# yhlleo/DWC-GAN

Hardware: AMD Instinct MI355X
Metric: CelebA 128x128 training images/sec (higher is better)
Workload: dtype f32; 1 GPU; BASELINE configs[1]: CelebA-shaped 128x128, per-GPU batch 16, fp32, full iteration (dis_update + gen_update + EMA + LR step), vgg_w=0, stride-1 3x3 / 5x5 and stride-2 4x4 layers (forward, data and weight gradient) as fp32-accurate TWO-plane f16 split products on the f16 MFMA (hi + lo 2^-11 per operand, per-tensor power-of-two scales, 3 products per multiply-add, matrix-core partial sums flushed to; image_size=128, per_gpu_batch=16, global_batch=16, parallelism=dp1

## Files before the change

### dwc-gan_amd/hipdwc/_lib.py

```python
import ctypes
import os

_HERE = os.path.dirname(os.path.abspath(__file__))
LIB_PATH = os.environ.get("DWC_HIP_LIB") or os.path.join(os.path.dirname(_HERE), "lib", "libdwcgan_hip.so")

c_fp = ctypes.c_void_p
c_int = ctypes.c_int
c_sz = ctypes.c_size_t
c_f = ctypes.c_float
c_u = ctypes.c_uint


class AdvSpec(ctypes.Structure):
    _fields_ = [("target", c_f * 4), ("w_src", c_f * 4), ("w_cls", c_f * 4)]


BN_MAX_SEGMENTS = 8


class BnOrder(ctypes.Structure):
    _fields_ = [("n", c_int), ("idx", c_int * BN_MAX_SEGMENTS)]


SIGNATURES = {
    "dwc_version": (c_int, []),
    "dwc_x3_gemm_mode": (c_int, [c_int]),
    "dwc_weight_prepared_elems": (c_sz, [c_int] * 8),
    "dwc_weight_prepare_fwd": (c_int, [c_fp, c_fp, c_int, c_int, c_int, c_int, c_int, c_int, c_fp]),
    "dwc_weight_prepare_dgrad": (c_int, [c_fp, c_fp, c_int, c_int, c_int, c_int, c_int, c_int, c_int, c_fp]),
    "dwc_conv2d_fwd_ws_bytes": (c_sz, [c_int] * 9),
    "dwc_conv2d_fwd": (c_int, [c_fp, c_fp, c_fp, c_fp] + [c_int] * 10 + [c_fp, c_sz, c_fp]),
    "dwc_conv2d_bwd_data_ws_bytes": (c_sz, [c_int] * 9),
# ... 183 lines not shown
    "dwc_bf16_conv2d_bwd_weight_plan": (c_int, [c_int] * 9 + [c_fp]),
    "dwc_conv2d_bwd_weight_zeropad_ws_bytes": (c_sz, [c_int] * 9),
    "dwc_conv2d_bwd_weight_zeropad": (c_int, [c_fp, c_fp, c_fp] + [c_int] * 11 + [c_fp, c_sz, c_fp]),
    "dwc_conv2d_bwd_data_crop_ws_bytes": (c_sz, [c_int] * 9),
    "dwc_conv2d_bwd_data_crop": (c_int, [c_fp, c_fp, c_fp] + [c_int] * 9 + [c_fp, c_sz, c_fp]),
    "dwc_bf16_conv2d_bwd_weight_zeropad_ws_bytes": (c_sz, [c_int] * 9),
    "dwc_bf16_conv2d_bwd_weight_zeropad": (c_int, [c_fp, c_fp, c_fp] + [c_int] * 11 + [c_fp, c_sz, c_fp]),
    "dwc_bf16_conv2d_bwd_data_crop_ws_bytes": (c_sz, [c_int] * 9),
    "dwc_bf16_conv2d_bwd_data_crop": (c_int, [c_fp, c_fp, c_fp] + [c_int] * 9 + [c_fp, c_sz, c_fp]),
    "dwc_x3_conv2d_wgrad_zeropad": (c_int, [c_fp, c_fp, c_fp] + [c_int] * 8 + [c_fp, c_sz, c_fp]),
    "dwc_h2_conv2d_wgrad_zeropad": (c_int, [c_fp, c_fp, c_u, c_fp, c_fp, c_u, c_fp] + [c_int] * 8 + [c_fp, c_sz, c_fp]),
    "dwc_bf16_conv2d_wgrad_halo_zeropad": (c_int, [c_fp, c_fp, c_fp] + [c_int] * 8 + [c_fp, c_sz, c_fp]),
    "dwc_x3_conv2d_s2_ws_zeropad": (c_int, [c_fp] * 4 + [c_int] * 7 + [c_fp, c_sz, c_fp, c_fp]),
    "dwc_h2_conv2d_s2_ws_zeropad": (c_int, [c_fp, c_fp, c_u, c_fp, c_fp, c_fp, c_fp, c_u] + [c_int] * 7 + [c_fp, c_sz, c_fp, c_fp]),
    "dwc_bf16_conv2d_s2_halo_zeropad": (c_int, [c_fp, c_fp, c_fp, c_fp] + [c_int] * 6 + [c_fp]),
}

ABI_VERSION = 11
EINVAL = -1
_ERRORS = {-1: "DWC_EINVAL (unsupported shape/argument)", -2: "DWC_EWORKSPACE (scratch too small)",
           -3: "DWC_ELAUNCH (kernel launch failed)"}

_lib = None


class HipKernelError(RuntimeError):
    pass


def load():
# ... 35 lines not shown
```

### dwc-gan_amd/hipdwc/ops.py

```python
import os
import weakref

import numpy as np
import torch

from . import _lib

ACT = {"none": 0, None: 0, "relu": 1, "lrelu": 2, "tanh": 3, "sigmoid": 4, "heads": 5, "heads8": 6}

PRECISION = "fp32"
BF16 = torch.bfloat16

_REMOVED_SWITCHES = ("DWC_WINOGRAD", "DWC_TXT_STREAM", "DWC_NORM_FUSED_FINAL", "DWC_GEMM_TILE", "DWC_STRIP_BM", "DWC_X3_DUO", "DWC_X3_BN",
                     "DWC_X3_BN32", "DWC_X3_WIDE", "DWC_X3_STAGGER", "DWC_HALO_STAGGER", "DWC_X3_WDUO", "DWC_HALO16", "DWC_HALO_DUO",
                     "DWC_HALO_BN128", "DWC_BF16_TILE", "DWC_BF16_STAGES3", "DWC_NARROW_ROWS16")
_set = [k for k in _REMOVED_SWITCHES if k in os.environ]
if _set:
    import warnings
    warnings.warn("hipdwc: %s no longer select%s anything (removed in round 5, DESIGN.md 10.3) and %s ignored" % (
        ", ".join(_set), "s" if len(_set) == 1 else "", "is" if len(_set) == 1 else "are"), stacklevel=2)
del _set


def set_precision(name):
# ... 1433 lines not shown
    K = w.shape[1]
    c = _pow2_div(N)
    taps = N // c
    wt4 = w.detach().t().reshape(K, taps, c).permute(0, 2, 1).unsqueeze(3)
    wp = _prepped(wt4, "fwd", K, c, 1, owner)
    dx = torch.empty((M, K), dtype=torch.float32, device=dy.device)
    nws = lib.dwc_conv2d_fwd_ws_bytes(M, taps, 1, c, K, taps, 1, 1, 0)
    wsp = workspace(nws, dy.device).data_ptr() if nws else None
    flops = 2.0 * M * N * K
    _lib.check(_timed("conv_gemm_kernel", flops, lambda: lib.dwc_conv2d_fwd(
        dy.data_ptr(), wp.data_ptr(), None, dx.data_ptr(), M, taps, 1, c, K, taps, 1, 1, 0, 0, wsp, nws, _stream()),
        detail="dgrad B%d %dx1 %d>%d k%d s1" % (M, taps, c, K, taps)), "gemm_nn")
    return dx


def _gemm_tn(dy, x, out=None):
    lib = _lib.load()
    M, N = dy.shape
    K = x.shape[1]
    c = _pow2_div(K)
    taps = K // c
    dw4 = torch.empty((N, c, 1, taps), dtype=torch.float32, device=x.device)
    nws = lib.dwc_conv2d_bwd_weight_ws_bytes(M, 1, taps, c, N, 1, taps, 1, 0)
    ws = workspace(nws, x.device)
    flops = 2.0 * M * N * K
    _lib.check(_timed("conv_wgrad_kernel+reduce", flops, lambda: lib.dwc_conv2d_bwd_weight(
        x.data_ptr(), dy.data_ptr(), dw4.data_ptr(), M, 1, taps, c, N, 1, taps, 1, 0, c, N, ws.data_ptr(), ws.numel(), _stream()),
        detail="wgrad B%d 1x%d %d>%d k%d s1" % (M, taps, c, N, taps)), "gemm_tn")
    if out is None:
        return dw4.squeeze(2).permute(0, 2, 1).reshape(N, K)
    out.view(N, taps, c).copy_(dw4.squeeze(2).permute(0, 2, 1))
    return out


class _LinearAny(torch.autograd.Function):

    @staticmethod
    def forward(ctx, x, w, b, owner):
        _require_device(x)
        if x.dtype != torch.float32 or not gemm_ok(x.shape[1], w.shape[0]):
            raise ValueError("linear_any: fp32, widths multiples of 4 (got %s x %s)" % (tuple(x.shape), tuple(w.shape)))
        x = x.contiguous()
        ctx.owner = owner if owner is not None else w
# ... 3 lines not shown

    @staticmethod
    def backward(ctx, dy):
        x, w = ctx.saved_tensors
        dy = dy.contiguous()
        dx = _gemm_nn(dy, w, ctx.owner) if ctx.needs_input_grad[0] else None
        dw = _gemm_tn(dy, x) if ctx.needs_input_grad[1] else None
        db = dy.sum(0) if (ctx.has_b and ctx.needs_input_grad[2]) else None
        return dx, dw, db, None


def linear_any(x, w, b, owner=None):
    return _LinearAny.apply(x, w, b, owner)


LSTM_GEMM = int(os.environ.get("DWC_LSTM_GEMM", "1"))
_LSTM_STATUS = {}
LSTM_SEQ_MAX_WORKGROUPS = 0


def _lstm_status(device):
    key = device.index if device.index is not None else torch.cuda.current_device()
    ent = _LSTM_STATUS.get(key)
    if ent is None:
        ent = [torch.zeros(1, dtype=torch.int32, device=device), torch.zeros(1, dtype=torch.int32).pin_memory(), None]
        _LSTM_STATUS[key] = ent
    return ent


def lstm_status_poll(device, wait=False):
# ... 2 lines not shown
    ent = _lstm_status(device)
    if ent[2] is not None and (wait or ent[2].query()):
        if wait:
            ent[2].synchronize()
        if int(ent[1][0]) != 0:
            raise _lib.HipKernelError(
                "persistent LSTM kernel: a workgroup hand-off timed out (status %d: not all workgroups of the launch were resident); "
                "its results were overwritten with NaN.  Re-run with DWC_LSTM_SEQ=0 (per-step kernels)." % int(ent[1][0]))
        ent[2] = None
    if ent[2] is None:
        ent[1].copy_(ent[0], non_blocking=True)
        ent[2] = torch.cuda.Event()
        ent[2].record()


class _LSTMBidir(torch.autograd.Function):

    @staticmethod
    def forward(ctx, x, lens, w_ih, w_hh, b_ih, b_hh, owners=None):
        _require_device(x)
        lib = _lib.load()
        T, B, I = x.shape
        H = w_hh.shape[2]
        dev = x.device
        X = x.reshape(T * B, I)
        ctx.hip_gemm = bool(LSTM_GEMM and owners is not None and gemm_ok(I, 4 * H) and gemm_ok(H, 4 * H))
        ctx.owners = owners
        if ctx.hip_gemm:
            bsum = b_ih + b_hh
            X = X.contiguous()
            xproj = torch.empty((2, T * B, 4 * H), dtype=torch.float32, device=dev)
            for d in range(2):
                _gemm_nt(X, w_ih[d], bsum[d], owners[d], out=xproj[d])
        else:
            xproj = torch.baddbmm((b_ih + b_hh).unsqueeze(1), X.unsqueeze(0).expand(2, -1, -1), w_ih.transpose(1, 2))
        w_hh_c = w_hh.contiguous()
        out = torch.empty((2, T, B, H), dtype=torch.float32, device=dev)
        c = torch.empty((2, T, B, H), dtype=torch.float32, device=dev)
        gates = torch.empty((2, T, B, 4 * H), dtype=torch.float32, device=dev)
        rc = -1
        if LSTM_SEQ:
            ws = workspace(lib.dwc_lstm_seq_ws_bytes(B, 2), dev)
            rc = lib.dwc_lstm_seq_fwd(xproj.data_ptr(), w_hh_c.data_ptr(), lens.data_ptr(), out.data_ptr(), c.data_ptr(),
                                      gates.data_ptr(), T, B, H, 2, ws.data_ptr(), ws.numel(), _lstm_status(dev)[0].data_ptr(),
                                      LSTM_SEQ_MAX_WORKGROUPS, _stream())
            if rc not in (0, _lib.EINVAL):
                _lib.check(rc, "lstm_seq_fwd")
        if rc != 0:
            _lib.check(lib.dwc_lstm_fwd(xproj.data_ptr(), w_hh_c.data_ptr(), lens.data_ptr(), out.data_ptr(), c.data_ptr(),
                                        gates.data_ptr(), T, B, H, 2, _stream()), "lstm_fwd")
        ctx.save_for_backward(X, lens, w_ih, w_hh_c, out, c, gates)
        ctx.shape = (T, B, I, H)
        return out, c

    @staticmethod
    def backward(ctx, d_out, d_c):
        lib = _lib.load()
        X, lens, w_ih, w_hh, out, c, gates = ctx.saved_tensors
        T, B, I, H = ctx.shape
        dev = X.device
        d_out = None if d_out is None else d_out.contiguous()
        d_c = None if d_c is None else d_c.contiguous()
        w_hh_t = w_hh.transpose(1, 2).contiguous()
        dgates = torch.empty((2, T, B, 4 * H), dtype=torch.float32, device=dev)
        carry = torch.empty((2, B, H), dtype=torch.float32, device=dev)
        rc = -1
        if LSTM_SEQ:
            ws = workspace(lib.dwc_lstm_seq_ws_bytes(B, 2), dev)
            rc = lib.dwc_lstm_seq_bwd(_p(d_out), _p(d_c), w_hh_t.data_ptr(), lens.data_ptr(), c.data_ptr(), gates.data_ptr(),
                                      dgates.data_ptr(), T, B, H, 2, ws.data_ptr(), ws.numel(), _lstm_status(dev)[0].data_ptr(),
                                      LSTM_SEQ_MAX_WORKGROUPS, _stream())
            if rc not in (0, _lib.EINVAL):
                _lib.check(rc, "lstm_seq_bwd")
        if rc != 0:
            _lib.check(lib.dwc_lstm_bwd(_p(d_out), _p(d_c), w_hh_t.data_ptr(), lens.data_ptr(), c.data_ptr(), gates.data_ptr(),
                                        dgates.data_ptr(), carry.data_ptr(), T, B, H, 2, _stream()), "lstm_bwd")
        dG = dgates.view(2, T * B, 4 * H)
        dGt = dG.transpose(1, 2)
        hip = ctx.hip_gemm
        dw_ih = None
        if ctx.needs_input_grad[2]:
            if hip:
                dw_ih = torch.empty((2, 4 * H, I), dtype=torch.float32, device=dev)
                for d in range(2):
                    _gemm_tn(dG[d], X, out=dw_ih[d])
            else:
                dw_ih = torch.matmul(dGt, X)
        db = dG.sum(1) if (ctx.needs_input_grad[4] or ctx.needs_input_grad[5]) else None
        dw_hh = None
        if ctx.needs_input_grad[3]:
            hprev = torch.zeros((2, T, B, H), dtype=torch.float32, device=dev)
            hprev[0, 1:] = out[0, :-1]
            hprev[1, :-1] = out[1, 1:]
            hp = hprev.view(2, T * B, H)
            if hip:
                dw_hh = torch.empty((2, 4 * H, H), dtype=torch.float32, device=dev)
                for d in range(2):
                    _gemm_tn(dG[d], hp[d], out=dw_hh[d])
            else:
                dw_hh = torch.bmm(dGt, hp)
        dx = None
        if ctx.needs_input_grad[0]:
            if hip:
                dx = (_gemm_nn(dG[0], w_ih[0], ctx.owners[0]) + _gemm_nn(dG[1], w_ih[1], ctx.owners[1])).view(T, B, I)
            else:
                dx = torch.bmm(dG, w_ih).sum(0).view(T, B, I)
        return dx, None, dw_ih, dw_hh, db, db, None


def lstm_bidir(x, lens, w_ih, w_hh, b_ih, b_hh, owners=None):
    return _LSTMBidir.apply(x.contiguous(), lens, w_ih, w_hh, b_ih, b_hh, owners)


def _norm_call(name, x, out, args):
    lib = _lib.load()
    slot, ep = out_amax(out)
    if slot is None:
        _lib.check(_fn(lib, name, x)(*args, _stream()), name)
        return None
    _lib.check(getattr(lib, "dwc_%s_amax" % name)(*args, slot, ep, _stream()), name)
    return slot, ep


class _InstNorm(torch.autograd.Function):
    @staticmethod
    def forward(ctx, x, gamma, beta, residual, act, eps, token=None):
# ... 355 lines not shown
```

### dwc-gan_amd/networks/networks_v2.py

```python
import numpy as np
import torch
from torch import nn

from hipdwc import host, ops
from .networks import ContentEncoder, MLP, Conv2dBlock, ResBlocks, AdaptiveInstanceNorm2d, Decoder


class HeadList(list):
    flat = None

    @classmethod
    def of(cls, flat, k):
        out = cls(flat.reshape(flat.shape[0], k, -1).unbind(1))
        out.flat = flat
        return out

    def rows(self, a, b):
        return HeadList.of(self.flat[a:b], len(self))


def flat_heads(heads):
    if torch.is_tensor(heads):
        return heads
    flat = getattr(heads, "flat", None)
# ... 76 lines not shown
            table = np.zeros((vocab.size, embed_dim))
            for i, word in enumerate(vocab.itos):
                table[i] = pretrained_embed[word] if word in pretrained_embed else \
                    np.random.normal(scale=0.6, size=(embed_dim,))
            self.embed_tokens.load_state_dict({"weight": torch.from_numpy(table)})
            self.embed_tokens.weight.requires_grad = False
        self.lstm = nn.LSTM(input_size=embed_dim + self.style_dim, hidden_size=hidden_size, num_layers=num_layers,
                            dropout=dropout_out if num_layers > 1 else 0.0, bidirectional=bidirectional)
        feat = hidden_size * num_layers * (4 if bidirectional else 2)
        self.fcs, self.fcvars = nn.ModuleList(), nn.ModuleList()
        for _ in range(num_class):
            self.fcs.append(nn.Linear(feat, c_dim))
            self.fcvars.append(nn.Linear(feat, c_dim))

    def forward(self, style_ord, src_tokens, src_lengths):
        noise = host.noise()
        tokens = src_tokens.transpose(1, 0)
        seq_len, bsz = tokens.shape
        lens_host = src_lengths.detach().to("cpu")
        lens_sorted, order_host = torch.sort(lens_host, descending=True)
        if tokens.is_cuda and ops.PINNED_STAGE:
            stage = torch.empty(4, bsz, dtype=torch.int64).pin_memory()
            stage[0], stage[1], stage[2], stage[3] = order_host, torch.sort(order_host)[1], lens_sorted, lens_sorted - 1
            on_dev = stage.to(tokens.device, non_blocking=True)
            order, unsort, lens_dev, last = on_dev[0], on_dev[1], on_dev[2].to(torch.int32), on_dev[3]
        else:
            order, unsort = order_host.to(tokens.device), torch.sort(order_host)[1].to(tokens.device)
            lens_dev, last = lens_sorted.to(torch.int32).to(tokens.device), (lens_sorted - 1).to(tokens.device)
        emb = self.embed_tokens(tokens.index_select(1, order))
        emb = noise.dropout(emb, self.dropout_in, self.training)
        sty = _Permute.apply(style_ord, 0, order, unsort)
        lens_list = lens_sorted.tolist()
        t_max = int(lens_list[0])
        data = torch.cat([emb, sty.expand(seq_len, -1, -1)], -1)[:t_max]
        cols = torch.arange(bsz, device=tokens.device)
        suffixes = ("", "_reverse") if self.bidirectional else ("",)
        if not self.bidirectional:
            raise NotImplementedError("the HIP text encoder is bidirectional (the reference's only configuration)")
        hs, cs = [], []
        for l in range(self.num_layers):
            par = {n: ops.cat_params([getattr(self.lstm, "%s_l%d%s" % (n, l, suf)) for suf in suffixes], stack=True)
                   for n in ("weight_ih", "weight_hh", "bias_ih", "bias_hh")}
            out, cell = ops.lstm_bidir(data, lens_dev, par["weight_ih"], par["weight_hh"], par["bias_ih"], par["bias_hh"],
                                       owners=tuple(getattr(self.lstm, "weight_ih_l%d%s" % (l, suf)) for suf in suffixes))
            hs += [out[0][last, cols], out[1][0]]
            cs += [cell[0][last, cols], cell[1][0]]
            data = torch.cat([out[0], out[1]], -1)
            if l + 1 < self.num_layers and self.training and self.dropout_out > 0:
                if getattr(noise, "align_stream", False):
                    mask = noise.dropout_mask((int(sum(lens_list)), data.shape[2]), self.dropout_out, data.device)
                    data = data * mask.index_select(0, _packed_index(lens_list, t_max, bsz, data.device)).view(t_max, bsz, -1)
                else:
                    data = noise.dropout(data, self.dropout_out, True)
        h_n, c_n = torch.stack(hs), torch.stack(cs)
        if self.training and self.dropout_out > 0 and noise.align_stream:
            noise.dropout(data, self.dropout_out, True)
        h_n = h_n.view(self.num_layers, 2, bsz, -1).transpose(1, 2).reshape(self.num_layers, bsz, -1)
        c_n = c_n.view(self.num_layers, 2, bsz, -1).transpose(1, 2).reshape(self.num_layers, bsz, -1)
        h_n, c_n = _Permute.apply(h_n, 1, unsort, order), _Permute.apply(c_n, 1, unsort, order)
        feat = torch.cat([h_n, c_n], dim=1).view(bsz, -1)
        w = ops.cat_params([m.weight for m in self.fcs] + [m.weight for m in self.fcvars])
        b = ops.cat_params([m.bias for m in self.fcs] + [m.bias for m in self.fcvars])
        if feat.is_cuda and ops.LSTM_GEMM and ops.gemm_ok(feat.shape[1], w.shape[0]):
            out = ops.linear_any(feat, w, b, owner=tuple(m.weight for m in self.fcs) + tuple(m.weight for m in self.fcvars))
        else:
            out = torch.nn.functional.linear(feat, w, b)
        k, c = self.num_class, self.style_dim // self.num_class
        return HeadList.of(out[:, :k * c], k), HeadList.of(out[:, k * c:2 * k * c], k)


class AdaINGen_v2(nn.Module):

    def __init__(self, input_dim, vocab, params, pretrained_embed=None):
        super().__init__()
        p = params
# ... 58 lines not shown
```

### include/dwcgan_hip.h

```cpp
#ifndef DWCGAN_HIP_H
#define DWCGAN_HIP_H

#include <stddef.h>
#include <stdint.h>

#ifdef __cplusplus
extern "C" {
#endif

#define DWC_OK 0
#define DWC_EINVAL (-1)
#define DWC_EWORKSPACE (-2)
#define DWC_ELAUNCH (-3)

#define DWC_ACT_NONE 0
#define DWC_ACT_RELU 1
#define DWC_ACT_LRELU 2
#define DWC_ACT_TANH 3
#define DWC_ACT_SIGMOID 4
#define DWC_ACT_HEADS 5
#define DWC_ACT_HEADS8 6

#define DWC_ABI_VERSION 11
int dwc_version(void);
// ... 413 lines not shown
                      float* dx, float* dgamma, float* dbeta, int S, int Bs, int HW, int C, int act, int training, void* ws,
                      size_t ws_bytes, void* stream);
int dwc_batchnorm_fwd_amax(const float* x, const float* gamma, const float* beta, float* running_mean, float* running_var, float* y,
                           float* mean, float* rstd, int S, int Bs, int HW, int C, float eps, float momentum, int act, int training,
                           dwc_bn_order order, void* ws, size_t ws_bytes, void* out_amax, unsigned out_epoch, void* stream);
int dwc_batchnorm_bwd_amax(const float* dy, const float* x, const float* mean, const float* rstd, const float* gamma,
                           const float* beta, float* dx, float* dgamma, float* dbeta, int S, int Bs, int HW, int C, int act,
                           int training, void* ws, size_t ws_bytes, void* out_amax, unsigned out_epoch, void* stream);
int dwc_bf16_batchnorm_fwd(const void* x, const float* gamma, const float* beta, float* running_mean, float* running_var, void* y,
                           float* mean, float* rstd, int S, int Bs, int HW, int C, float eps, float momentum, int act, int training,
                           dwc_bn_order order, void* ws, size_t ws_bytes, void* stream);
int dwc_bf16_batchnorm_bwd(const void* dy, const void* x, const float* mean, const float* rstd, const float* gamma,
                           const float* beta, void* dx, float* dgamma, float* dbeta, int S, int Bs, int HW, int C, int act,
                           int training, void* ws, size_t ws_bytes, void* stream);

#ifdef __cplusplus
}
#endif
#endif
```

Baseline: 398.2 images/s.

## Fuse text-encoder LSTM glue into HIP kernels with a custom autograd stack

```diff
diff --git a/dwc-gan_amd/csrc/txt_glue.hip b/dwc-gan_amd/csrc/txt_glue.hip
--- /dev/null
+++ b/dwc-gan_amd/csrc/txt_glue.hip
@@ -0,0 +1,195 @@
+#include "dwc_common.h"
+
+namespace {
+
+__device__ __forceinline__ int txt_perm(const int* __restrict__ perm, int k, int B) { return min(max(perm[k], 0), B - 1); }
+
+__global__ __launch_bounds__(256) void txt_operand_fwd_kernel(const float* __restrict__ table, const long long* __restrict__ tokens,
+                                                              const int* __restrict__ order, const float* __restrict__ mask,
+                                                              const float* __restrict__ style, float* __restrict__ X, int B,
+                                                              int seq_len, int E, int S, int vocab) {
+    const int row = blockIdx.x, t = row / B, j = row - t * B;
+    const int src = txt_perm(order, j, B);
+    const long long tok = tokens[(size_t)src * seq_len + t];
+    const bool ok = tok >= 0 && tok < vocab;
+    const float* e = table + (size_t)(ok ? tok : 0) * E;
+    const float* m = mask ? mask + (size_t)row * E : nullptr;
+    float* x = X + (size_t)row * (E + S);
+    for (int k = threadIdx.x; k < E; k += 256) {
+        const float v = m ? e[k] * m[k] : e[k];
+        x[k] = ok ? v : __builtin_nanf("");
+    }
+    const float* s = style + (size_t)src * S;
+    for (int k = threadIdx.x; k < S; k += 256) x[E + k] = s[k];
+}
+
+__global__ __launch_bounds__(256) void txt_operand_bwd_kernel(const float* __restrict__ dxa, const float* __restrict__ dxb,
+                                                              const long long* __restrict__ tokens, const int* __restrict__ order,
+                                                              const float* __restrict__ mask, float* __restrict__ d_cat,
+                                                              float* __restrict__ d_emb, long long* __restrict__ idx, int t_max, int B,
+                                                              int seq_len, int E, int S) {
+    const int row = blockIdx.x, t = row / B, j = row - t * B, I = E + S;
+    const int src = txt_perm(order, j, B);
+    const bool live = t < t_max;
+    const size_t in = (size_t)row * I;
+    if (d_emb) {
+        const float* m = mask ? mask + (size_t)row * E : nullptr;
+        for (int k = threadIdx.x; k < E; k += 256) {
+            float g = 0.f;
+            if (live) {
+                g = dxb ? dxa[in + k] + dxb[in + k] : dxa[in + k];
+                if (m) g = __fmul_rn(g, m[k]);
+            }
+            d_emb[(size_t)row * E + k] = g;
+        }
+    }
+    if (d_cat) {
+        float* o = d_cat + ((size_t)t * B + src) * I + E;
+        for (int k = threadIdx.x; k < S; k += 256) o[k] = live ? (dxb ? dxa[in + E + k] + dxb[in + E + k] : dxa[in + E + k]) : 0.f;
+    }
+    if (idx && threadIdx.x == 0) idx[row] = tokens[(size_t)src * seq_len + t];
+}
+
+__global__ __launch_bounds__(256) void txt_prev_state_kernel(const float* __restrict__ out, float* __restrict__ hprev, int T, int B, int H) {
+    const int row = blockIdx.x, d = blockIdx.y, t = row / B;
+    const int tp = d == 0 ? t - 1 : t + 1;
+    const bool has = tp >= 0 && tp < T;
+    const float* src = out + ((size_t)d * T * B + (size_t)(has ? tp : t) * B + (row - t * B)) * H;
+    float* dst = hprev + ((size_t)d * T * B + row) * H;
+    for (int u = threadIdx.x; u < H; u += 256) dst[u] = has ? src[u] : 0.f;
+}
+
+__global__ __launch_bounds__(256) void txt_inter_fwd_kernel(const float* __restrict__ out, const float* __restrict__ mask,
+                                                            const long long* __restrict__ mask_row, float* __restrict__ data, int T,
+                                                            int B, int H) {
+    const size_t row = blockIdx.x, TB = (size_t)T * B;
+    const float* m = mask ? mask + (size_t)(mask_row ? mask_row[row] : (long long)row) * 2 * H : nullptr;
+    for (int k = threadIdx.x; k < 2 * H; k += 256) {
+        const int d = k >= H, u = k - d * H;
+        const float v = out[(d * TB + row) * H + u];
+        data[row * 2 * H + k] = m ? v * m[k] : v;
+    }
+}
+
+__device__ __forceinline__ bool txt_is_final(int d, int t, int last_j) { return t == (d == 0 ? last_j : 0); }
+__device__ __forceinline__ size_t txt_feat_at(int l, int is_c, int caller_row, int d, int u, int B, int H) {
+    return ((((size_t)l * 2 + is_c) * B + caller_row) * 2 + d) * H + u;
+}
+
+__global__ __launch_bounds__(256) void txt_states_fwd_kernel(dwc_txt_layers ly, const int* __restrict__ last,
+                                                             const int* __restrict__ unsort, float* __restrict__ feat, int T, int B,
+                                                             int H) {
+    const int i = blockIdx.x, l = blockIdx.y >> 1, is_c = blockIdx.y & 1;
+    const int j = txt_perm(unsort, i, B);
+    const float* src = is_c ? ly.c[l] : ly.out[l];
+    const int t_fwd = min(max(last[j], 0), T - 1);
+    for (int k = threadIdx.x; k < 2 * H; k += 256) {
+        const int d = k >= H, u = k - d * H;
+        const int t = d == 0 ? t_fwd : 0;
+        feat[txt_feat_at(l, is_c, i, d, u, B, H)] = src[(((size_t)d * T + t) * B + j) * H + u];
+    }
+}
+
+__global__ __launch_bounds__(256) void txt_states_bwd_kernel(const float* __restrict__ d_feat, const int* __restrict__ order,
+                                                             const int* __restrict__ last, dwc_txt_layers ly, int T, int B, int H) {
+    const int l = blockIdx.z >> 1, is_c = blockIdx.z & 1, d = blockIdx.y;
+    float* dst = is_c ? ly.c[l] : ly.out[l];
+    if (!dst) return;
+    const int row = blockIdx.x, t = row / B, j = row - t * B;
+    const bool fin = txt_is_final(d, t, last[j]);
+    const int i = txt_perm(order, j, B);
+    float* o = dst + ((size_t)d * T * B + row) * H;
+    for (int u = threadIdx.x; u < H; u += 256) o[u] = fin ? d_feat[txt_feat_at(l, is_c, i, d, u, B, H)] : 0.f;
+}
+
+__global__ __launch_bounds__(256) void txt_inter_bwd_kernel(const float* __restrict__ dxa, const float* __restrict__ dxb,
+                                                            const float* __restrict__ mask, const long long* __restrict__ mask_row,
+                                                            const float* __restrict__ d_feat, const int* __restrict__ order,
+                                                            const int* __restrict__ last, int l, float* __restrict__ d_out, int T,
+                                                            int B, int H) {
+    const int row = blockIdx.x, d = blockIdx.y, t = row / B, j = row - t * B;
+    const float* m = mask ? mask + (size_t)(mask_row ? mask_row[row] : (long long)row) * 2 * H + d * H : nullptr;
+    const bool fin = txt_is_final(d, t, last[j]);
+    const int i = txt_perm(order, j, B);
+    const size_t in = (size_t)row * 2 * H + d * H;
+    float* o = d_out + ((size_t)d * T * B + row) * H;
+    for (int u = threadIdx.x; u < H; u += 256) {
+        float g = dxb ? dxa[in + u] + dxb[in + u] : dxa[in + u];
+        if (m) g = __fmul_rn(g, m[u]);
+        o[u] = fin ? g + d_feat[txt_feat_at(l, 0, i, d, u, B, H)] : g;
+    }
+}
+
+bool txt_layers_ok(const dwc_txt_layers& ly) { return ly.n >= 1 && ly.n <= DWC_TXT_MAX_LAYERS; }
+
+}
+
+extern "C" {
+
+int dwc_txt_operand_fwd(const float* table, const long long* tokens, const int* order, const float* mask, const float* style,
+                        float* x, int t_max, int B, int seq_len, int E, int S, int vocab, void* stream) {
+    if (!table || !tokens || !order || !x || (S > 0 && !style) || t_max < 1 || t_max > seq_len || B < 1 || E < 1 || S < 0 || vocab < 1)
+        return DWC_EINVAL;
+    hipLaunchKernelGGL(txt_operand_fwd_kernel, dim3(t_max * B), dim3(256), 0, (hipStream_t)stream, table, tokens, order, mask, style, x,
+                       B, seq_len, E, S, vocab);
+    DWC_LAUNCH_CHECK();
+    return DWC_OK;
+}
+
+int dwc_txt_operand_bwd(const float* dxa, const float* dxb, const long long* tokens, const int* order, const float* mask,
+                        float* d_cat, float* d_emb, long long* idx, int t_max, int B, int seq_len, int E, int S, void* stream) {
+    if (!dxa || !tokens || !order || (!d_cat && !d_emb && !idx) || t_max < 1 || t_max > seq_len || B < 1 || E < 1 || S < 0 ||
+        (d_cat && S < 1) || (long long)seq_len * B > 0x7fffffffLL)
+        return DWC_EINVAL;
+    hipLaunchKernelGGL(txt_operand_bwd_kernel, dim3(seq_len * B), dim3(256), 0, (hipStream_t)stream, dxa, dxb, tokens, order, mask,
+                       d_cat, d_emb, idx, t_max, B, seq_len, E, S);
+    DWC_LAUNCH_CHECK();
+    return DWC_OK;
+}
+
+int dwc_txt_prev_state(const float* out, float* hprev, int T, int B, int H, void* stream) {
+    if (!out || !hprev || T < 1 || B < 1 || H < 1 || (long long)T * B > 0x7fffffffLL) return DWC_EINVAL;
+    hipLaunchKernelGGL(txt_prev_state_kernel, dim3(T * B, 2), dim3(256), 0, (hipStream_t)stream, out, hprev, T, B, H);
+    DWC_LAUNCH_CHECK();
+    return DWC_OK;
+}
+
+int dwc_txt_inter_fwd(const float* out, const float* mask, const long long* mask_row, float* data, int T, int B, int H, void* stream) {
+    if (!out || !data || (mask_row && !mask) || T < 1 || B < 1 || H < 1) return DWC_EINVAL;
+    hipLaunchKernelGGL(txt_inter_fwd_kernel, dim3(T * B), dim3(256), 0, (hipStream_t)stream, out, mask, mask_row, data, T, B, H);
+    DWC_LAUNCH_CHECK();
+    return DWC_OK;
+}
+
+int dwc_txt_inter_bwd(const float* dxa, const float* dxb, const float* mask, const long long* mask_row, const float* d_feat,
+                      const int* order, const int* last, int layer, float* d_out, int T, int B, int H, void* stream) {
+    if (!dxa || !d_feat || !order || !last || !d_out || (mask_row && !mask) || layer < 0 || layer >= DWC_TXT_MAX_LAYERS || T < 1 ||
+        B < 1 || H < 1)
+        return DWC_EINVAL;
+    hipLaunchKernelGGL(txt_inter_bwd_kernel, dim3(T * B, 2), dim3(256), 0, (hipStream_t)stream, dxa, dxb, mask, mask_row, d_feat, order,
+                       last, layer, d_out, T, B, H);
+    DWC_LAUNCH_CHECK();
+    return DWC_OK;
+}
+
+int dwc_txt_states_fwd(dwc_txt_layers layers, const int* last, const int* unsort, float* feat, int T, int B, int H, void* stream) {
+    if (!txt_layers_ok(layers) || !last || !unsort || !feat || T < 1 || B < 1 || H < 1) return DWC_EINVAL;
+    for (int l = 0; l < layers.n; ++l)
+        if (!layers.out[l] || !layers.c[l]) return DWC_EINVAL;
+    hipLaunchKernelGGL(txt_states_fwd_kernel, dim3(B, 2 * layers.n), dim3(256), 0, (hipStream_t)stream, layers, last, unsort, feat, T, B,
+                       H);
+    DWC_LAUNCH_CHECK();
+    return DWC_OK;
+}
+
+int dwc_txt_states_bwd(const float* d_feat, const int* order, const int* last, dwc_txt_layers grads, int T, int B, int H,
+                       void* stream) {
+    if (!txt_layers_ok(grads) || !d_feat || !order || !last || T < 1 || B < 1 || H < 1 || (long long)T * B > 0x7fffffffLL)
+        return DWC_EINVAL;
+    hipLaunchKernelGGL(txt_states_bwd_kernel, dim3(T * B, 2, 2 * grads.n), dim3(256), 0, (hipStream_t)stream, d_feat, order, last, grads,
+                       T, B, H);
+    DWC_LAUNCH_CHECK();
+    return DWC_OK;
+}
+
+}
diff --git a/dwc-gan_amd/hipdwc/_lib.py b/dwc-gan_amd/hipdwc/_lib.py
--- a/dwc-gan_amd/hipdwc/_lib.py
+++ b/dwc-gan_amd/hipdwc/_lib.py
@@ -16,6 +16,13 @@
 
 
 BN_MAX_SEGMENTS = 8
+
+
+TXT_MAX_LAYERS = 4
+
+
+class TxtLayers(ctypes.Structure):
+    _fields_ = [("n", c_int), ("out", c_fp * TXT_MAX_LAYERS), ("c", c_fp * TXT_MAX_LAYERS)]
 
 
 class BnOrder(ctypes.Structure):
@@ -229,6 +236,13 @@
     "dwc_x3_conv2d_s2_ws_zeropad": (c_int, [c_fp] * 4 + [c_int] * 7 + [c_fp, c_sz, c_fp, c_fp]),
     "dwc_h2_conv2d_s2_ws_zeropad": (c_int, [c_fp, c_fp, c_u, c_fp, c_fp, c_fp, c_fp, c_u] + [c_int] * 7 + [c_fp, c_sz, c_fp, c_fp]),
     "dwc_bf16_conv2d_s2_halo_zeropad": (c_int, [c_fp, c_fp, c_fp, c_fp] + [c_int] * 6 + [c_fp]),
+    "dwc_txt_operand_fwd": (c_int, [c_fp] * 6 + [c_int] * 6 + [c_fp]),
+    "dwc_txt_operand_bwd": (c_int, [c_fp] * 8 + [c_int] * 5 + [c_fp]),
+    "dwc_txt_prev_state": (c_int, [c_fp, c_fp] + [c_int] * 3 + [c_fp]),
+    "dwc_txt_inter_fwd": (c_int, [c_fp] * 4 + [c_int] * 3 + [c_fp]),
+    "dwc_txt_inter_bwd": (c_int, [c_fp] * 7 + [c_int, c_fp] + [c_int] * 3 + [c_fp]),
+    "dwc_txt_states_fwd": (c_int, [TxtLayers, c_fp, c_fp, c_fp] + [c_int] * 3 + [c_fp]),
+    "dwc_txt_states_bwd": (c_int, [c_fp, c_fp, c_fp, TxtLayers] + [c_int] * 3 + [c_fp]),
 }
 
 ABI_VERSION = 11
diff --git a/dwc-gan_amd/hipdwc/ops.py b/dwc-gan_amd/hipdwc/ops.py
--- a/dwc-gan_amd/hipdwc/ops.py
+++ b/dwc-gan_amd/hipdwc/ops.py
@@ -1471,19 +1471,23 @@
     return dx
 
 
-def _gemm_tn(dy, x, out=None):
+def _gemm_tn(dy, x, out=None, raw=None):
     lib = _lib.load()
     M, N = dy.shape
     K = x.shape[1]
     c = _pow2_div(K)
     taps = K // c
-    dw4 = torch.empty((N, c, 1, taps), dtype=torch.float32, device=x.device)
+    if raw is not None:
+        assert raw.shape == (N, c, taps) and raw.is_contiguous() and raw.dtype == torch.float32
+    dw4 = torch.empty((N, c, 1, taps), dtype=torch.float32, device=x.device) if raw is None else raw
     nws = lib.dwc_conv2d_bwd_weight_ws_bytes(M, 1, taps, c, N, 1, taps, 1, 0)
     ws = workspace(nws, x.device)
     flops = 2.0 * M * N * K
     _lib.check(_timed("conv_wgrad_kernel+reduce", flops, lambda: lib.dwc_conv2d_bwd_weight(
         x.data_ptr(), dy.data_ptr(), dw4.data_ptr(), M, 1, taps, c, N, 1, taps, 1, 0, c, N, ws.data_ptr(), ws.numel(), _stream()),
         detail="wgrad B%d 1x%d %d>%d k%d s1" % (M, taps, c, N, taps)), "gemm_tn")
+    if raw is not None:
+        return raw
     if out is None:
         return dw4.squeeze(2).permute(0, 2, 1).reshape(N, K)
     out.view(N, taps, c).copy_(dw4.squeeze(2).permute(0, 2, 1))
@@ -1517,6 +1521,7 @@
     return _LinearAny.apply(x, w, b, owner)
 
 
+TXT_FUSED = int(os.environ.get("DWC_TXT_FUSED", "1"))
 LSTM_GEMM = int(os.environ.get("DWC_LSTM_GEMM", "1"))
 _LSTM_STATUS = {}
 LSTM_SEQ_MAX_WORKGROUPS = 0
@@ -1549,102 +1554,141 @@
         ent[2].record()
 
 
+_LSTM_DERIVED = {}
+
+
+def _stamp(params):
+    return None if params is None else tuple((p._version, p.data_ptr()) for p in params)
+
+
+def _lstm_derived(kind, owners, stamp, build):
+    if owners is None:
+        return build()
+    key = (kind, id(owners[0]))
+    ent = _LSTM_DERIVED.get(key)
+    if ent is not None and ent[0]() is owners[0] and ent[1] == stamp:
+        return ent[2]
+    buf = build()
+    _LSTM_DERIVED[key] = (weakref.ref(owners[0], lambda _r, key=key: _LSTM_DERIVED.pop(key, None)), stamp, buf)
+    return buf
+
+
+def lstm_layer_fwd(x, lens, w_ih, w_hh, b_ih, b_hh, owners=None, owners_hh=None, owners_b=None):
+    _require_device(x)
+    lib = _lib.load()
+    T, B, I = x.shape
+    H = w_hh.shape[2]
+    dev = x.device
+    X = x.reshape(T * B, I)
+    hip_gemm = bool(LSTM_GEMM and owners is not None and gemm_ok(I, 4 * H) and gemm_ok(H, 4 * H))
+    if hip_gemm:
+        bsum = _lstm_derived("bsum", owners_b, _stamp(owners_b), lambda: b_ih.detach() + b_hh.detach())
+        X = X.contiguous()
+        xproj = torch.empty((2, T * B, 4 * H), dtype=torch.float32, device=dev)
+        for d in range(2):
+            _gemm_nt(X, w_ih[d], bsum[d], owners[d], out=xproj[d])
+    else:
+        xproj = torch.baddbmm((b_ih + b_hh).unsqueeze(1), X.unsqueeze(0).expand(2, -1, -1), w_ih.transpose(1, 2))
+    w_hh_c = w_hh.contiguous()
+    out = torch.empty((2, T, B, H), dtype=torch.float32, device=dev)
+    c = torch.empty((2, T, B, H), dtype=torch.float32, device=dev)
+    gates = torch.empty((2, T, B, 4 * H), dtype=torch.float32, device=dev)
+    rc = -1
+    if LSTM_SEQ:
+        ws = workspace(lib.dwc_lstm_seq_ws_bytes(B, 2), dev)
+        rc = lib.dwc_lstm_seq_fwd(xproj.data_ptr(), w_hh_c.data_ptr(), lens.data_ptr(), out.data_ptr(), c.data_ptr(),
+                                  gates.data_ptr(), T, B, H, 2, ws.data_ptr(), ws.numel(), _lstm_status(dev)[0].data_ptr(),
+                                  LSTM_SEQ_MAX_WORKGROUPS, _stream())
+        if rc not in (0, _lib.EINVAL):
+            _lib.check(rc, "lstm_seq_fwd")
+    if rc != 0:
+        _lib.check(lib.dwc_lstm_fwd(xproj.data_ptr(), w_hh_c.data_ptr(), lens.data_ptr(), out.data_ptr(), c.data_ptr(),
+                                    gates.data_ptr(), T, B, H, 2, _stream()), "lstm_fwd")
+    saved = {"tensors": (X, lens, w_ih, w_hh_c, out, c, gates), "shape": (T, B, I, H), "hip_gemm": hip_gemm, "owners": owners,
+             "owners_hh": owners_hh, "hh_stamp": _stamp(owners_hh)}
+    return out, c, saved
+
+
+def lstm_layer_bwd(saved, d_out, d_c, need_x=True, need_w_ih=True, need_w_hh=True, need_b=True, split_dx=False):
+    lib = _lib.load()
+    X, lens, w_ih, w_hh, out, c, gates = saved["tensors"]
+    T, B, I, H = saved["shape"]
+    dev = X.device
+    d_out = None if d_out is None else d_out.contiguous()
+    d_c = None if d_c is None else d_c.contiguous()
+    w_hh_t = _lstm_derived("w_hh_t", saved["owners_hh"], saved["hh_stamp"], lambda: w_hh.transpose(1, 2).contiguous())
+    dgates = torch.empty((2, T, B, 4 * H), dtype=torch.float32, device=dev)
+    carry = torch.empty((2, B, H), dtype=torch.float32, device=dev)
+    rc = -1
+    if LSTM_SEQ:
+        ws = workspace(lib.dwc_lstm_seq_ws_bytes(B, 2), dev)
+        rc = lib.dwc_lstm_seq_bwd(_p(d_out), _p(d_c), w_hh_t.data_ptr(), lens.data_ptr(), c.data_ptr(), gates.data_ptr(),
+                                  dgates.data_ptr(), T, B, H, 2, ws.data_ptr(), ws.numel(), _lstm_status(dev)[0].data_ptr(),
+                                  LSTM_SEQ_MAX_WORKGROUPS, _stream())
+        if rc not in (0, _lib.EINVAL):
+            _lib.check(rc, "lstm_seq_bwd")
+    if rc != 0:
+        _lib.check(lib.dwc_lstm_bwd(_p(d_out), _p(d_c), w_hh_t.data_ptr(), lens.data_ptr(), c.data_ptr(), gates.data_ptr(),
+                                    dgates.data_ptr(), carry.data_ptr(), T, B, H, 2, _stream()), "lstm_bwd")
+    dG = dgates.view(2, T * B, 4 * H)
+    dGt = dG.transpose(1, 2)
+    hip = saved["hip_gemm"]
+
+    def relaid(raw, K):
+        return raw.transpose(2, 3).reshape(2, 4 * H, K)
+
+    dw_ih = None
+    if need_w_ih:
+        if hip:
+            raw = torch.empty((2, 4 * H, _pow2_div(I), I // _pow2_div(I)), dtype=torch.float32, device=dev)
+            for d in range(2):
+                _gemm_tn(dG[d], X, raw=raw[d])
+            dw_ih = relaid(raw, I)
+        else:
+            dw_ih = torch.matmul(dGt, X)
+    db = dG.sum(1) if need_b else None
+    dw_hh = None
+    if need_w_hh:
+        hprev = torch.empty((2, T, B, H), dtype=torch.float32, device=dev)
+        _lib.check(lib.dwc_txt_prev_state(out.data_ptr(), hprev.data_ptr(), T, B, H, _stream()), "txt_prev_state")
+        hp = hprev.view(2, T * B, H)
+        if hip:
+            raw = torch.empty((2, 4 * H, _pow2_div(H), H // _pow2_div(H)), dtype=torch.float32, device=dev)
+            for d in range(2):
+                _gemm_tn(dG[d], hp[d], raw=raw[d])
+            dw_hh = relaid(raw, H)
+        else:
+            dw_hh = torch.bmm(dGt, hp)
+    dx = None
+    if need_x:
+        if hip:
+            parts = (_gemm_nn(dG[0], w_ih[0], saved["owners"][0]).view(T, B, I), _gemm_nn(dG[1], w_ih[1], saved["owners"][1]).view(T, B, I))
+            dx = parts if split_dx else parts[0] + parts[1]
+        else:
+            dx = torch.bmm(dG, w_ih).sum(0).view(T, B, I)
+            dx = (dx, None) if split_dx else dx
+    return dx, dw_ih, dw_hh, db
+
+
 class _LSTMBidir(torch.autograd.Function):
 
     @staticmethod
-    def forward(ctx, x, lens, w_ih, w_hh, b_ih, b_hh, owners=None):
-        _require_device(x)
-        lib = _lib.load()
-        T, B, I = x.shape
-        H = w_hh.shape[2]
-        dev = x.device
-        X = x.reshape(T * B, I)
-        ctx.hip_gemm = bool(LSTM_GEMM and owners is not None and gemm_ok(I, 4 * H) and gemm_ok(H, 4 * H))
-        ctx.owners = owners
-        if ctx.hip_gemm:
-            bsum = b_ih + b_hh
-            X = X.contiguous()
-            xproj = torch.empty((2, T * B, 4 * H), dtype=torch.float32, device=dev)
-            for d in range(2):
-                _gemm_nt(X, w_ih[d], bsum[d], owners[d], out=xproj[d])
-        else:
-            xproj = torch.baddbmm((b_ih + b_hh).unsqueeze(1), X.unsqueeze(0).expand(2, -1, -1), w_ih.transpose(1, 2))
-        w_hh_c = w_hh.contiguous()
-        out = torch.empty((2, T, B, H), dtype=torch.float32, device=dev)
-        c = torch.empty((2, T, B, H), dtype=torch.float32, device=dev)
-        gates = torch.empty((2, T, B, 4 * H), dtype=torch.float32, device=dev)
-        rc = -1
-        if LSTM_SEQ:
-            ws = workspace(lib.dwc_lstm_seq_ws_bytes(B, 2), dev)
-            rc = lib.dwc_lstm_seq_fwd(xproj.data_ptr(), w_hh_c.data_ptr(), lens.data_ptr(), out.data_ptr(), c.data_ptr(),
-                                      gates.data_ptr(), T, B, H, 2, ws.data_ptr(), ws.numel(), _lstm_status(dev)[0].data_ptr(),
-                                      LSTM_SEQ_MAX_WORKGROUPS, _stream())
-            if rc not in (0, _lib.EINVAL):
-                _lib.check(rc, "lstm_seq_fwd")
-        if rc != 0:
-            _lib.check(lib.dwc_lstm_fwd(xproj.data_ptr(), w_hh_c.data_ptr(), lens.data_ptr(), out.data_ptr(), c.data_ptr(),
-                                        gates.data_ptr(), T, B, H, 2, _stream()), "lstm_fwd")
-        ctx.save_for_backward(X, lens, w_ih, w_hh_c, out, c, gates)
-        ctx.shape = (T, B, I, H)
+    def forward(ctx, x, lens, w_ih, w_hh, b_ih, b_hh, owners=None, owners_hh=None, owners_b=None):
+        out, c, saved = lstm_layer_fwd(x, lens, w_ih, w_hh, b_ih, b_hh, owners, owners_hh, owners_b)
+        ctx.save_for_backward(*saved.pop("tensors"))
+        ctx.saved = saved
         return out, c
 
     @staticmethod
     def backward(ctx, d_out, d_c):
-        lib = _lib.load()
-        X, lens, w_ih, w_hh, out, c, gates = ctx.saved_tensors
-        T, B, I, H = ctx.shape
-        dev = X.device
-        d_out = None if d_out is None else d_out.contiguous()
-        d_c = None if d_c is None else d_c.contiguous()
-        w_hh_t = w_hh.transpose(1, 2).contiguous()
-        dgates = torch.empty((2, T, B, 4 * H), dtype=torch.float32, device=dev)
-        carry = torch.empty((2, B, H), dtype=torch.float32, device=dev)
-        rc = -1
-        if LSTM_SEQ:
-            ws = workspace(lib.dwc_lstm_seq_ws_bytes(B, 2), dev)
-            rc = lib.dwc_lstm_seq_bwd(_p(d_out), _p(d_c), w_hh_t.data_ptr(), lens.data_ptr(), c.data_ptr(), gates.data_ptr(),
-                                      dgates.data_ptr(), T, B, H, 2, ws.data_ptr(), ws.numel(), _lstm_status(dev)[0].data_ptr(),
-                                      LSTM_SEQ_MAX_WORKGROUPS, _stream())
-            if rc not in (0, _lib.EINVAL):
-                _lib.check(rc, "lstm_seq_bwd")
-        if rc != 0:
-            _lib.check(lib.dwc_lstm_bwd(_p(d_out), _p(d_c), w_hh_t.data_ptr(), lens.data_ptr(), c.data_ptr(), gates.data_ptr(),
-                                        dgates.data_ptr(), carry.data_ptr(), T, B, H, 2, _stream()), "lstm_bwd")
-        dG = dgates.view(2, T * B, 4 * H)
-        dGt = dG.transpose(1, 2)
-        hip = ctx.hip_gemm
-        dw_ih = None
-        if ctx.needs_input_grad[2]:
-            if hip:
-                dw_ih = torch.empty((2, 4 * H, I), dtype=torch.float32, device=dev)
-                for d in range(2):
-                    _gemm_tn(dG[d], X, out=dw_ih[d])
-            else:
-                dw_ih = torch.matmul(dGt, X)
-        db = dG.sum(1) if (ctx.needs_input_grad[4] or ctx.needs_input_grad[5]) else None
-        dw_hh = None
-        if ctx.needs_input_grad[3]:
-            hprev = torch.zeros((2, T, B, H), dtype=torch.float32, device=dev)
-            hprev[0, 1:] = out[0, :-1]
-            hprev[1, :-1] = out[1, 1:]
-            hp = hprev.view(2, T * B, H)
-            if hip:
-                dw_hh = torch.empty((2, 4 * H, H), dtype=torch.float32, device=dev)
-                for d in range(2):
-                    _gemm_tn(dG[d], hp[d], out=dw_hh[d])
-            else:
-                dw_hh = torch.bmm(dGt, hp)
-        dx = None
-        if ctx.needs_input_grad[0]:
-            if hip:
-                dx = (_gemm_nn(dG[0], w_ih[0], ctx.owners[0]) + _gemm_nn(dG[1], w_ih[1], ctx.owners[1])).view(T, B, I)
-            else:
-                dx = torch.bmm(dG, w_ih).sum(0).view(T, B, I)
-        return dx, None, dw_ih, dw_hh, db, db, None
-
-
-def lstm_bidir(x, lens, w_ih, w_hh, b_ih, b_hh, owners=None):
-    return _LSTMBidir.apply(x.contiguous(), lens, w_ih, w_hh, b_ih, b_hh, owners)
+        saved = dict(ctx.saved, tensors=ctx.saved_tensors)
+        need = ctx.needs_input_grad
+        dx, dw_ih, dw_hh, db = lstm_layer_bwd(saved, d_out, d_c, need[0], need[2], need[3], need[4] or need[5])
+        return dx, None, dw_ih, dw_hh, db, db, None, None, None
+
+
+def lstm_bidir(x, lens, w_ih, w_hh, b_ih, b_hh, owners=None, owners_hh=None, owners_b=None):
+    return _LSTMBidir.apply(x.contiguous(), lens, w_ih, w_hh, b_ih, b_hh, owners, owners_hh, owners_b)
 
 
 def _norm_call(name, x, out, args):
diff --git a/dwc-gan_amd/hipdwc/txt.py b/dwc-gan_amd/hipdwc/txt.py
--- /dev/null
+++ b/dwc-gan_amd/hipdwc/txt.py
@@ -0,0 +1,206 @@
+import torch
+
+from . import _lib, host, ops
+from .ops import _p, _stream
+
+MAX_LAYERS = _lib.TXT_MAX_LAYERS
+
+
+def _f32(t, shape=None):
+    assert t.is_cuda and t.dtype == torch.float32 and t.is_contiguous(), "dense fp32 device tensor expected"
+    assert shape is None or tuple(t.shape) == tuple(shape), (tuple(t.shape), tuple(shape))
+    return t
+
+
+def _i32(t, n):
+    assert t.is_cuda and t.dtype == torch.int32 and t.is_contiguous() and t.numel() == n, "int32 [%d] device tensor expected" % n
+    return t
+
+
+def _layers(outs, cs):
+    ly = _lib.TxtLayers()
+    ly.n = len(outs)
+    for l, (o, c) in enumerate(zip(outs, cs)):
+        ly.out[l], ly.c[l] = _p(o), _p(c)
+    return ly
+
+
+def operand_fwd(table, tokens, order, mask, style, t_max):
+    B, seq_len = tokens.shape
+    V, E = table.shape
+    S = style.shape[1]
+    assert tokens.dtype == torch.int64 and tokens.is_contiguous() and 1 <= t_max <= seq_len
+    assert mask is None or (_f32(mask).shape[0] >= t_max and mask.shape[1:] == (B, E))
+    x = torch.empty((t_max, B, E + S), dtype=torch.float32, device=table.device)
+    _lib.check(_lib.load().dwc_txt_operand_fwd(_f32(table).data_ptr(), tokens.data_ptr(), _i32(order, B).data_ptr(), _p(mask),
+                                               _f32(style, (B, S)).data_ptr(), x.data_ptr(), t_max, B, seq_len, E, S, V, _stream()),
+               "txt_operand_fwd")
+    return x
+
+
+def operand_bwd(dxa, dxb, tokens, order, mask, E, vocab, padding_idx, need_style=True, need_table=True):
+    t_max, B, I = dxa.shape
+    S = I - E
+    seq_len = tokens.shape[1]
+    _f32(dxa)
+    assert dxb is None or _f32(dxb).shape == dxa.shape
+    if not (need_style or need_table):
+        return None, None
+    dev = dxa.device
+    d_cat = torch.empty((seq_len, B, I), dtype=torch.float32, device=dev) if need_style else None
+    d_emb = torch.empty((seq_len, B, E), dtype=torch.float32, device=dev) if need_table else None
+    idx = torch.empty((seq_len, B), dtype=torch.int64, device=dev) if need_table else None
+    _lib.check(_lib.load().dwc_txt_operand_bwd(dxa.data_ptr(), _p(dxb), tokens.data_ptr(), _i32(order, B).data_ptr(), _p(mask),
+                                               _p(d_cat), _p(d_emb), _p(idx), t_max, B, seq_len, E, S, _stream()), "txt_operand_bwd")
+    d_style = d_cat[:, :, E:].sum(0) if need_style else None
+    d_table = None
+    if need_table:
+        d_table = torch.ops.aten.embedding_dense_backward(d_emb, idx, vocab, -1 if padding_idx is None else int(padding_idx), False)
+    return d_style, d_table
+
+
+def _mask_args(mask, mask_row, T, B, H):
+    if mask is None:
+        return None, None
+    if mask_row is None:
+        _f32(mask, (T, B, 2 * H))
+        return mask.data_ptr(), None
+    assert _f32(mask).dim() == 2 and mask.shape[1] == 2 * H
+    assert mask_row.is_cuda and mask_row.dtype == torch.int64 and mask_row.is_contiguous() and mask_row.numel() == T * B
+    return mask.data_ptr(), mask_row.data_ptr()
+
+
+def inter_fwd(out, mask=None, mask_row=None):
+    _, T, B, H = _f32(out).shape
+    m, r = _mask_args(mask, mask_row, T, B, H)
+    data = torch.empty((T, B, 2 * H), dtype=torch.float32, device=out.device)
+    _lib.check(_lib.load().dwc_txt_inter_fwd(out.data_ptr(), m, r, data.data_ptr(), T, B, H, _stream()), "txt_inter_fwd")
+    return data
+
+
+def inter_bwd(dxa, dxb, mask, mask_row, d_feat, order, last, layer, H):
+    T, B, _ = _f32(dxa, (dxa.shape[0], dxa.shape[1], 2 * H)).shape
+    assert dxb is None or _f32(dxb).shape == dxa.shape
+    m, r = _mask_args(mask, mask_row, T, B, H)
+    assert _f32(d_feat).numel() % (4 * B * H) == 0 and 0 <= layer < d_feat.numel() // (4 * B * H)
+    d_out = torch.empty((2, T, B, H), dtype=torch.float32, device=dxa.device)
+    _lib.check(_lib.load().dwc_txt_inter_bwd(dxa.data_ptr(), _p(dxb), m, r, d_feat.data_ptr(), _i32(order, B).data_ptr(),
+                                             _i32(last, B).data_ptr(), layer, d_out.data_ptr(), T, B, H, _stream()), "txt_inter_bwd")
+    return d_out
+
+
+def states_fwd(outs, cs, last, unsort):
+    L = len(outs)
+    assert 1 <= L <= MAX_LAYERS and len(cs) == L
+    _, T, B, H = outs[0].shape
+    for t in list(outs) + list(cs):
+        _f32(t, (2, T, B, H))
+    feat = torch.empty((B, 4 * L * H), dtype=torch.float32, device=outs[0].device)
+    _lib.check(_lib.load().dwc_txt_states_fwd(_layers(outs, cs), _i32(last, B).data_ptr(), _i32(unsort, B).data_ptr(), feat.data_ptr(),
+                                              T, B, H, _stream()), "txt_states_fwd")
+    return feat
+
+
+def states_bwd(d_feat, order, last, T, H, need_out):
+    B = d_feat.shape[0]
+    L = d_feat.shape[1] // (4 * H)
+    assert 1 <= L <= MAX_LAYERS and _f32(d_feat).shape[1] == 4 * L * H and len(need_out) == L
+    new = lambda: torch.empty((2, T, B, H), dtype=torch.float32, device=d_feat.device)
+    d_outs = [new() if need_out[l] else None for l in range(L)]
+    d_cs = [new() for _ in range(L)]
+    _lib.check(_lib.load().dwc_txt_states_bwd(d_feat.data_ptr(), _i32(order, B).data_ptr(), _i32(last, B).data_ptr(),
+                                              _layers(d_outs, d_cs), T, B, H, _stream()), "txt_states_bwd")
+    return d_outs, d_cs
+
+
+class _Plan:
+    __slots__ = ("tokens", "order", "unsort", "lens", "last", "t_max", "mask_in", "masks", "mask_rows", "owners_ih", "owners_hh", "owners_b",
+                 "padding_idx", "layers")
+
+
+class _TxtStack(torch.autograd.Function):
+
+    @staticmethod
+    def forward(ctx, plan, table, style, *params):
+        data = operand_fwd(table, plan.tokens, plan.order, plan.mask_in, style.contiguous(), plan.t_max)
+        outs, cs, saved = [], [], []
+        for l in range(plan.layers):
+            out, c, sv = ops.lstm_layer_fwd(data, plan.lens, *params[4 * l:4 * l + 4], owners=plan.owners_ih[l],
+                                            owners_hh=plan.owners_hh[l], owners_b=plan.owners_b[l])
+            outs.append(out)
+            cs.append(c)
+            saved.append(sv)
+            if l + 1 < plan.layers:
+                data = inter_fwd(out, plan.masks[l], plan.mask_rows[l])
+        ctx.save_for_backward(*[t for sv in saved for t in sv.pop("tensors")])
+        ctx.plan, ctx.saved = plan, saved
+        ctx.table_shape = tuple(table.shape)
+        return states_fwd(outs, cs, plan.last, plan.unsort)
+
+    @staticmethod
+    def backward(ctx, d_feat):
+        plan, L = ctx.plan, ctx.plan.layers
+        kept = ctx.saved_tensors
+        saved = [dict(sv, tensors=kept[l * len(kept) // L:(l + 1) * len(kept) // L]) for l, sv in enumerate(ctx.saved)]
+        T, _, _, H = saved[0]["shape"]
+        need = ctx.needs_input_grad
+        d_feat = d_feat.contiguous()
+        d_outs, d_cs = states_bwd(d_feat, plan.order, plan.last, T, H, [l == L - 1 for l in range(L)])
+        d_out = d_outs[L - 1]
+        grads = [None] * (4 * L)
+        d_style = d_table = None
+        for l in reversed(range(L)):
+            nw = need[3 + 4 * l:7 + 4 * l]
+            need_x = l > 0 or need[1] or need[2]
+            dx, dw_ih, dw_hh, db = ops.lstm_layer_bwd(saved[l], d_out, d_cs[l], need_x, nw[0], nw[1], nw[2] or nw[3], split_dx=True)
+            grads[4 * l:4 * l + 4] = [dw_ih, dw_hh, db, db]
+            if l > 0:
+                d_out = inter_bwd(dx[0], dx[1], plan.masks[l - 1], plan.mask_rows[l - 1], d_feat, plan.order, plan.last, l - 1, H)
+            elif need_x:
+                d_style, d_table = operand_bwd(dx[0], dx[1], plan.tokens, plan.order, plan.mask_in, ctx.table_shape[1],
+                                               ctx.table_shape[0], plan.padding_idx, need_style=need[2], need_table=need[1])
+        return (None, d_table, d_style) + tuple(grads)
+
+
+def encode(enc, style_ord, src_tokens, src_lengths, packed_index):
+    if enc.num_layers > MAX_LAYERS:
+        raise ValueError("the text encoder's kernels take up to %d LSTM layers (DWC_TXT_MAX_LAYERS), got %d" % (MAX_LAYERS, enc.num_layers))
+    noise = host.noise()
+    dev = src_tokens.device
+    bsz, seq_len = src_tokens.shape
+    lens_sorted, order_host = torch.sort(src_lengths.detach().to("cpu"), descending=True)
+    stage = torch.empty(4, bsz, dtype=torch.int32)
+    if ops.PINNED_STAGE:
+        stage = stage.pin_memory()
+    stage[0], stage[1], stage[2], stage[3] = order_host, torch.sort(order_host)[1], lens_sorted, lens_sorted - 1
+    on_dev = stage.to(dev, non_blocking=True)
+    lens_list = lens_sorted.tolist()
+    training = enc.training
+    H, E = enc.hidden_size, enc.embed_dim
+
+    plan = _Plan()
+    plan.tokens = src_tokens.long().contiguous()
+    plan.order, plan.unsort, plan.lens, plan.last = on_dev[0], on_dev[1], on_dev[2], on_dev[3]
+    plan.t_max, plan.layers, plan.padding_idx = int(lens_list[0]), enc.num_layers, enc.embed_tokens.padding_idx
+    plan.mask_in = noise.dropout_mask((seq_len, bsz, E), enc.dropout_in, dev) if training and enc.dropout_in > 0 else None
+    plan.masks, plan.mask_rows = [], []
+    for l in range(enc.num_layers - 1):
+        mask = rows = None
+        if training and enc.dropout_out > 0:
+            if getattr(noise, "align_stream", False):
+                mask = noise.dropout_mask((int(sum(lens_list)), 2 * H), enc.dropout_out, dev)
+                rows = packed_index(lens_list, plan.t_max, bsz, dev)
+            else:
+                mask = noise.dropout_mask((plan.t_max, bsz, 2 * H), enc.dropout_out, dev)
+        plan.masks.append(mask)
+        plan.mask_rows.append(rows)
+    if training and enc.dropout_out > 0 and getattr(noise, "align_stream", False):
+        noise.dropout_mask((plan.t_max, bsz, 2 * H), enc.dropout_out, dev)
+    names = ("weight_ih", "weight_hh", "bias_ih", "bias_hh")
+    per_layer = [{n: tuple(getattr(enc.lstm, "%s_l%d%s" % (n, l, suf)) for suf in ("", "_reverse")) for n in names}
+                 for l in range(enc.num_layers)]
+    plan.owners_ih = [p["weight_ih"] for p in per_layer]
+    plan.owners_hh = [p["weight_hh"] for p in per_layer]
+    plan.owners_b = [p["bias_ih"] + p["bias_hh"] for p in per_layer]
+    params = [ops.cat_params(p[n], stack=True) for p in per_layer for n in names]
+    return _TxtStack.apply(plan, enc.embed_tokens.weight, style_ord, *params)
diff --git a/dwc-gan_amd/networks/networks_v2.py b/dwc-gan_amd/networks/networks_v2.py
--- a/dwc-gan_amd/networks/networks_v2.py
+++ b/dwc-gan_amd/networks/networks_v2.py
@@ -2,7 +2,7 @@
 import torch
 from torch import nn
 
-from hipdwc import host, ops
+from hipdwc import host, ops, txt
 from .networks import ContentEncoder, MLP, Conv2dBlock, ResBlocks, AdaptiveInstanceNorm2d, Decoder
 
 
@@ -114,6 +114,10 @@
             self.fcvars.append(nn.Linear(feat, c_dim))
 
     def forward(self, style_ord, src_tokens, src_lengths):
+        if not self.bidirectional:
+            raise NotImplementedError("the HIP text encoder is bidirectional (the reference's only configuration)")
+        if ops.TXT_FUSED and src_tokens.is_cuda:
+            return self._heads(txt.encode(self, style_ord, src_tokens, src_lengths, _packed_index))
         noise = host.noise()
         tokens = src_tokens.transpose(1, 0)
         seq_len, bsz = tokens.shape
@@ -134,15 +138,16 @@
         t_max = int(lens_list[0])
         data = torch.cat([emb, sty.expand(seq_len, -1, -1)], -1)[:t_max]
         cols = torch.arange(bsz, device=tokens.device)
-        suffixes = ("", "_reverse") if self.bidirectional else ("",)
-        if not self.bidirectional:
-            raise NotImplementedError("the HIP text encoder is bidirectional (the reference's only configuration)")
+        suffixes = ("", "_reverse")
         hs, cs = [], []
         for l in range(self.num_layers):
             par = {n: ops.cat_params([getattr(self.lstm, "%s_l%d%s" % (n, l, suf)) for suf in suffixes], stack=True)
                    for n in ("weight_ih", "weight_hh", "bias_ih", "bias_hh")}
             out, cell = ops.lstm_bidir(data, lens_dev, par["weight_ih"], par["weight_hh"], par["bias_ih"], par["bias_hh"],
-                                       owners=tuple(getattr(self.lstm, "weight_ih_l%d%s" % (l, suf)) for suf in suffixes))
+                                       owners=tuple(getattr(self.lstm, "weight_ih_l%d%s" % (l, suf)) for suf in suffixes),
+                                       owners_hh=tuple(getattr(self.lstm, "weight_hh_l%d%s" % (l, suf)) for suf in suffixes),
+                                       owners_b=tuple(getattr(self.lstm, "%s_l%d%s" % (n, l, suf)) for n in ("bias_ih", "bias_hh")
+                                                      for suf in suffixes))
             hs += [out[0][last, cols], out[1][0]]
             cs += [cell[0][last, cols], cell[1][0]]
             data = torch.cat([out[0], out[1]], -1)
@@ -158,7 +163,9 @@
         h_n = h_n.view(self.num_layers, 2, bsz, -1).transpose(1, 2).reshape(self.num_layers, bsz, -1)
         c_n = c_n.view(self.num_layers, 2, bsz, -1).transpose(1, 2).reshape(self.num_layers, bsz, -1)
         h_n, c_n = _Permute.apply(h_n, 1, unsort, order), _Permute.apply(c_n, 1, unsort, order)
-        feat = torch.cat([h_n, c_n], dim=1).view(bsz, -1)
+        return self._heads(torch.cat([h_n, c_n], dim=1).view(bsz, -1))
+
+    def _heads(self, feat):
         w = ops.cat_params([m.weight for m in self.fcs] + [m.weight for m in self.fcvars])
         b = ops.cat_params([m.bias for m in self.fcs] + [m.bias for m in self.fcvars])
         if feat.is_cuda and ops.LSTM_GEMM and ops.gemm_ok(feat.shape[1], w.shape[0]):
diff --git a/include/dwcgan_hip.h b/include/dwcgan_hip.h
--- a/include/dwcgan_hip.h
+++ b/include/dwcgan_hip.h
@@ -451,6 +451,24 @@
                            const float* beta, void* dx, float* dgamma, float* dbeta, int S, int Bs, int HW, int C, int act,
                            int training, void* ws, size_t ws_bytes, void* stream);
 
+int dwc_txt_operand_fwd(const float* table, const long long* tokens, const int* order, const float* mask, const float* style,
+                        float* x, int t_max, int B, int seq_len, int E, int S, int vocab, void* stream);
+int dwc_txt_operand_bwd(const float* dxa, const float* dxb, const long long* tokens, const int* order, const float* mask,
+                        float* d_cat, float* d_emb, long long* idx, int t_max, int B, int seq_len, int E, int S, void* stream);
+int dwc_txt_prev_state(const float* out, float* hprev, int T, int B, int H, void* stream);
+int dwc_txt_inter_fwd(const float* out, const float* mask, const long long* mask_row, float* data, int T, int B, int H, void* stream);
+int dwc_txt_inter_bwd(const float* dxa, const float* dxb, const float* mask, const long long* mask_row, const float* d_feat,
+                      const int* order, const int* last, int layer, float* d_out, int T, int B, int H, void* stream);
+#define DWC_TXT_MAX_LAYERS 4
+typedef struct dwc_txt_layers {
+    int n;
+    float* out[DWC_TXT_MAX_LAYERS];
+    float* c[DWC_TXT_MAX_LAYERS];
+} dwc_txt_layers;
+int dwc_txt_states_fwd(dwc_txt_layers layers, const int* last, const int* unsort, float* feat, int T, int B, int H, void* stream);
+int dwc_txt_states_bwd(const float* d_feat, const int* order, const int* last, dwc_txt_layers grads, int T, int B, int H,
+                       void* stream);
+
 #ifdef __cplusplus
 }
 #endif
```

New measurement: 403.3 images/s (median of 6 runs). 1.3% higher.
